# pierrepaleo/sift_pyocl

Hardware: AMD Instinct MI355X
Metric: SiftPlan.keypoints throughput, 4096x4096 fp32 (Mpix/s; keypoints/s in keypoints_per_s) (higher is better)
Workload: dtype f32

## Files before the change

### sift_pyocl_amd/csrc/k_extrema.hpp

```cpp
#pragma once
#include <hip/hip_runtime.h>
#include <stdint.h>
#include "siftmath.hpp"
#include "k_xcd.hpp"
#include <type_traits>

namespace siftk {

struct BlurPlanes { const float *p[6]; };

#define SIFT_EXT_ROWS 64
inline int extrema_strip_rows(int W, int H, int border, int min_strips = 2000) {
    const int nx = (W - 2 * border + 61) / 62;
    int rows = SIFT_EXT_ROWS;
    while (rows > 4 && (int64_t)nx * ((H - 2 * border + rows - 1) / rows) < min_strips) rows >>= 1;
    return rows;
}

__device__ __forceinline__ float dog_at(const BlurPlanes &b, int s, size_t pos) { return b.p[s][pos] - b.p[s + 1][pos]; }

#ifndef SIFT_EXT_WAVES
#define SIFT_EXT_WAVES 5
#endif
#define SIFT_EXT_BUF 128
template <int BUF> struct ExtWaveLdsT { float4 buf[BUF + 192]; };
using ExtWaveLds = ExtWaveLdsT<SIFT_EXT_BUF>;

struct RefineArgs {
    float peak_thresh, init_sigma;
    float4 *kp;
    int *kp_aux, *n_kp;
    int kp_capacity, oct;
    int *c_scale;
};
__device__ __forceinline__ void refine_candidates(const BlurPlanes &b, int W, int H, const float4 *__restrict__ cand, int n,
                                                  float peak_thresh, float init_sigma, float4 *__restrict__ kp,
                                                  int *__restrict__ kp_aux, int *__restrict__ n_kp, int kp_capacity, int oct,
                                                  int first, int stride, int *__restrict__ c_scale);

template <int BUF>
__device__ __forceinline__ void ext_store_pending(const ExtWaveLdsT<BUF> &L, float4 *__restrict__ cand, int capacity, int slot, int count, int lane) {
    __builtin_amdgcn_wave_barrier();
    for (int e = lane; e < count; e += 64)
        if (slot + e < capacity) cand[slot + e] = L.buf[e];
    __builtin_amdgcn_wave_barrier();
}

template <int BUF>
__device__ __forceinline__ void ext_edge_filter(const BlurPlanes &b, int W, float edth, ExtWaveLdsT<BUF> &L, int from, int &pending, int lane) {
    int out = from;
    __builtin_amdgcn_wave_barrier();
    for (int base = from; base < pending; base += 64) {
        const int e = base + lane;
        bool keep = false;
        float4 c = make_float4(0.f, 0.f, 0.f, 0.f);
        if (e < pending) {
            c = L.buf[e];
            const float val = c.x;
            const int s = (int)c.w;
            const size_t pc = (size_t)(int)c.y * W + (int)c.z;
            const float *pa = b.p[1], *pb = b.p[2];
            if (s == 2) { pa = b.p[2]; pb = b.p[3]; } else if (s == 3) { pa = b.p[3]; pb = b.p[4]; }
#define DOG_AT(o) (pa[pc + (o)] - pb[pc + (o)])
            const float up = DOG_AT(-(ptrdiff_t)W), dn = DOG_AT(W);
            const float lf = DOG_AT(-1), rt = DOG_AT(1);
            const float H00 = (float)(((double)up - 2.0 * (double)val) + (double)dn);
            const float H11 = (float)(((double)lf - 2.0 * (double)val) + (double)rt);
            const float dd = (DOG_AT(W + 1) - DOG_AT(W - 1)) - (DOG_AT(-(ptrdiff_t)W + 1) - DOG_AT(-(ptrdiff_t)W - 1));
#undef DOG_AT
            const float H01 = (float)((double)dd / 4.0);
            const float det = H00 * H11 - H01 * H01;
            const float tr = H00 + H11;
            keep = !(det < edth * tr * tr) && val != 0.0f;
        }
        __builtin_amdgcn_wave_barrier();
        const unsigned long long m = __ballot(keep);
        if (keep) L.buf[out + __popcll(m & ((1ull << lane) - 1ull))] = c;
        out += __popcll(m);
        __builtin_amdgcn_wave_barrier();
    }
    pending = out;
}

template <int BUF, bool REFINE = false>
__device__ __forceinline__ void extrema_strip(const BlurPlanes &b, int W, int H, int border, int rows, bool active, int sx, int sy,
                                              double contrast, float edth, float4 *__restrict__ cand, int *__restrict__ counter,
                                              int capacity, ExtWaveLdsT<BUF> &L, int &pending, const RefineArgs *ra = nullptr,
                                              int y_lo = -1, int y_hi = -1) {
    if (y_lo < 0) { y_lo = border; y_hi = H - border; }
    auto refine_parked = [&]() {
        __builtin_amdgcn_wave_barrier();
        refine_candidates(b, W, H, L.buf, pending, ra->peak_thresh, ra->init_sigma, ra->kp, ra->kp_aux, ra->n_kp, ra->kp_capacity,
                          ra->oct, threadIdx.x & 63, 64, ra->c_scale);
        __builtin_amdgcn_wave_barrier();
        pending = 0;
    };
    const int lane = threadIdx.x & 63;
    const int x = border + sx * 62 + lane - 1;
    const int xc = min(max(x, 0), W - 1);
    const bool col_ok = (lane >= 1) && (lane <= 62) && (x < W - border);
    const int ya = y_lo + sy * rows;
    const int yb = active ? min(ya + rows, y_hi) : ya - 2;
    int tested = pending;

    float cf = (float)contrast;
    if (!((double)cf > contrast)) cf = __uint_as_float(__float_as_uint(cf) + 1u);
    auto ld = [&](int k, unsigned off) { return *reinterpret_cast<const float *>(reinterpret_cast<const char *>(b.p[k]) + off); };
    auto from_left = [](float v) { return __int_as_float(__builtin_amdgcn_update_dpp(0, __float_as_int(v), 0x138, 0xf, 0xf, true)); };
    auto from_right = [](float v) { return __int_as_float(__builtin_amdgcn_update_dpp(0, __float_as_int(v), 0x130, 0xf, 0xf, true)); };

    float hM[3][3], hm[3][3];
    float ctr[3] = {0.f, 0.f, 0.f}, ctr_next[3];
#pragma unroll
    for (int r = 0; r < 3; r++)
#pragma unroll
        for (int k = 0; k < 3; k++) { hM[r][k] = 0.f; hm[r][k] = 0.f; }

    const unsigned pitch = (unsigned)W * 4u;
    unsigned off = ((unsigned)max(ya - 1, 0) * (unsigned)W + (unsigned)xc) * 4u;
    float vn[6];
    if (active) {
#pragma unroll
        for (int k = 0; k < 6; k++) vn[k] = ld(k, off);
    } else {
#pragma unroll
        for (int k = 0; k < 6; k++) vn[k] = 0.f;
    }
    for (int y = ya - 1; y <= yb; y++) {
        float v[6];
#pragma unroll
        for (int k = 0; k < 6; k++) v[k] = vn[k];
        if (y < yb) {
            off += pitch;
#pragma unroll
            for (int k = 0; k < 6; k++) vn[k] = ld(k, off);
        }
        float d[5];
#pragma unroll
        for (int k = 0; k < 5; k++) d[k] = v[k] - v[k + 1];
#pragma unroll
        for (int k = 0; k < 3; k++) { hM[0][k] = hM[1][k]; hM[1][k] = hM[2][k]; hm[0][k] = hm[1][k]; hm[1][k] = hm[2][k]; }
#pragma unroll
        for (int k = 0; k < 3; k++) {
            const float M = fmaxf(fmaxf(d[k], d[k + 1]), d[k + 2]);
            const float m = fminf(fminf(d[k], d[k + 1]), d[k + 2]);
            hM[2][k] = fmaxf(fmaxf(from_left(M), M), from_right(M));
            hm[2][k] = fminf(fminf(from_left(m), m), from_right(m));
            ctr_next[k] = d[k + 1];
        }
        bool found[3] = {false, false, false};
        const int yc = y - 1;
        if (y >= ya + 1 && col_ok) {
#pragma unroll
            for (int k = 0; k < 3; k++) {
                const float val = ctr[k];
                if (fabsf(val) >= cf) {
                    const float M27 = fmaxf(fmaxf(hM[0][k], hM[1][k]), hM[2][k]);
                    const float m27 = fminf(fminf(hm[0][k], hm[1][k]), hm[2][k]);
                    found[k] = (val > 0.0f) ? (val >= M27) : (val <= m27);
                }
            }
        }
#pragma unroll
        for (int k = 0; k < 3; k++) {
            const unsigned long long m = __ballot(found[k]);
            if (m) {
                if (found[k]) L.buf[pending + __popcll(m & ((1ull << lane) - 1ull))] = make_float4(ctr[k], (float)yc, (float)x, (float)(k + 1));
                pending += __popcll(m);
            }
        }
        if (pending > BUF) {
            ext_edge_filter(b, W, edth, L, tested, pending, lane);
            tested = 0;
            if (REFINE) refine_parked();
            else {
                int slot = 0;
                if (lane == 0) slot = atomicAdd(counter, pending);
                ext_store_pending(L, cand, capacity, __shfl(slot, 0), pending, lane);
                pending = 0;
            }
        }
#pragma unroll
        for (int k = 0; k < 3; k++) ctr[k] = ctr_next[k];
    }
    ext_edge_filter(b, W, edth, L, tested, pending, lane);
    if (REFINE) refine_parked();
}

template <bool REFINE>
__global__ __launch_bounds__(256) __attribute__((amdgpu_waves_per_eu(REFINE ? 4 : SIFT_EXT_WAVES, 8))) void extrema_kernel(BlurPlanes b, int W, int H, int border, int rows, double contrast,
                                                      float edth, float4 *__restrict__ cand,
                                                      int *__restrict__ counter, int capacity, RefineArgs ra,
                                                      int y_lo, int y_hi,
                                                      int xcd_map) {
    __shared__ ExtWaveLds lds_all[4];
    __shared__ int s_pending[4], s_base;
    const int lane = threadIdx.x & 63;
    ExtWaveLds &L = lds_all[threadIdx.x >> 6];
    if (y_lo < 0) { y_lo = border; y_hi = H - border; }
    const int nx = (W - 2 * border + 61) / 62;
    const int ny = (y_hi - y_lo + rows - 1) / rows;
    const int wg = xcd_map ? xcd_contiguous((int)blockIdx.x, (int)gridDim.x) : (int)blockIdx.x;
    const int wid = wg * 4 + (threadIdx.x >> 6);
    const bool active = wid < nx * ny;
    int pending = 0;
    extrema_strip<SIFT_EXT_BUF, REFINE>(b, W, H, border, rows, active, active ? wid % nx : 0, active ? wid / nx : 0, contrast, edth, cand,
                                        counter, capacity, L, pending, &ra, y_lo, y_hi);
    if (REFINE) return;
    if (lane == 0) s_pending[threadIdx.x >> 6] = pending;
    __syncthreads();
    if (threadIdx.x == 0) {
        const int tot = s_pending[0] + s_pending[1] + s_pending[2] + s_pending[3];
        s_base = tot ? atomicAdd(counter, tot) : 0;
    }
    __syncthreads();
    {
        const int w = threadIdx.x >> 6;
        int slot = s_base;
        for (int q = 0; q < w; q++) slot += s_pending[q];
        ext_store_pending(L, cand, capacity, slot, pending, lane);
    }
}

__device__ __forceinline__ void refine_candidates(const BlurPlanes &b, int W, int H, const float4 *__restrict__ cand, int n,
                                                  float peak_thresh, float init_sigma, float4 *__restrict__ kp,
                                                  int *__restrict__ kp_aux, int *__restrict__ n_kp, int kp_capacity, int oct,
                                                  int first, int stride, int *__restrict__ c_scale) {
    int seen[3] = {0, 0, 0};
    for (int i = first; i < n; i += stride) {
        const float4 k = cand[i];
        int r = (int)k.y, c = (int)k.z;
        const int scale = (int)k.w;
        if (r == -1) continue;
        seen[0] += scale <= 1; seen[1] += scale == 2; seen[2] += scale >= 3;
        const float *Pa = b.p[0], *Pb = b.p[1], *Pc = b.p[2], *Pd = b.p[3];
        if (scale == 2) { Pa = b.p[1]; Pb = b.p[2]; Pc = b.p[3]; Pd = b.p[4]; }
        else if (scale == 3) { Pa = b.p[2]; Pb = b.p[3]; Pc = b.p[4]; Pd = b.p[5]; }
        int newr = r, newc = c, moves = 5;
        bool again = true;
        float s0 = 0.f, s1 = 0.f, s2 = 0.f, peak = 0.f;
        while (again) {
            r = newr; c = newc;
            const size_t pos = (size_t)r * W + c;
#define DOGP(o) (Pa[pos + (o)] - Pb[pos + (o)])
#define DOGD(o) (Pb[pos + (o)] - Pc[pos + (o)])
#define DOGN(o) (Pc[pos + (o)] - Pd[pos + (o)])
            const float P0 = DOGP(0), D0 = DOGD(0), N0 = DOGN(0);
            const float Dd = DOGD(W), Du = DOGD(-W), Dr = DOGD(1), Dl = DOGD(-1);
            const float Pd_ = DOGP(W), Pu = DOGP(-W), Pr = DOGP(1), Pl = DOGP(-1);
            const float Nd = DOGN(W), Nu = DOGN(-W), Nr = DOGN(1), Nl = DOGN(-1);
            const float Ddr = DOGD(W + 1), Ddl = DOGD(W - 1), Dur = DOGD(-W + 1), Dul = DOGD(-W - 1);
#undef DOGP
#undef DOGD
#undef DOGN
            const float g0 = (N0 - P0) / 2.0f;
            const float g1 = (Dd - Du) / 2.0f;
            const float g2 = (Dr - Dl) / 2.0f;
            const float H00 = P0 - 2.0f * D0 + N0;
            const float H11 = Du - 2.0f * D0 + Dd;
            const float H22 = Dl - 2.0f * D0 + Dr;
            const float H01 = ((Nd - Nu) - (Pd_ - Pu)) / 4.0f;
            const float H02 = ((Nr - Nl) - (Pr - Pl)) / 4.0f;
            const float H12 = ((Ddr - Ddl) - (Dur - Dul)) / 4.0f;
            const float H10 = H01, H20 = H02, H21 = H12;
            const float det = -(H02 * H11 * H20) + H01 * H12 * H20 + H02 * H10 * H21
                              - H00 * H12 * H21 - H01 * H10 * H22 + H00 * H11 * H22;
            const float K00 = H11 * H22 - H12 * H21;
            const float K01 = H02 * H21 - H01 * H22;
            const float K02 = H01 * H12 - H02 * H11;
            const float K10 = H12 * H20 - H10 * H22;
            const float K11 = H00 * H22 - H02 * H20;
            const float K12 = H02 * H10 - H00 * H12;
            const float K20 = H10 * H21 - H11 * H20;
            const float K21 = H01 * H20 - H00 * H21;
            const float K22 = H00 * H11 - H01 * H10;
            s0 = -(g0 * K00 + g1 * K01 + g2 * K02) / det;
            s1 = -(g0 * K10 + g1 * K11 + g2 * K12) / det;
            s2 = -(g0 * K20 + g1 * K21 + g2 * K22) / det;
            peak = D0 + 0.5f * (s0 * g0 + s1 * g1 + s2 * g2);
            if (s1 > 0.6f && newr < H - 3) newr++;
            else if (s1 < -0.6f && newr > 3) newr--;
            if (s2 > 0.6f && newc < W - 3) newc++;
            else if (s2 < -0.6f && newc > 3) newc--;
            if (moves > 0 && (newr != r || newc != c)) moves--;
            else again = false;
        }
        if (fabsf(s0) <= 1.5f && fabsf(s1) <= 1.5f && fabsf(s2) <= 1.5f && fabsf(peak) >= peak_thresh) {
            const float sig = init_sigma * siftmath::exp2f_(((float)scale + s0) / 3.0f);
            const int slot = atomicAdd(n_kp, 1);
            if (slot < kp_capacity) {
                kp[slot] = make_float4(peak, (float)r + s1, (float)c + s2, sig);
                kp_aux[slot] = scale | (oct << 8);
            }
        }
    }
    if (c_scale) {
#pragma unroll
        for (int q = 0; q < 3; q++) {
            int t = seen[q];
#pragma unroll
            for (int off = 32; off > 0; off >>= 1) t += __shfl_xor(t, off);
            if (t && (threadIdx.x & 63) == q) atomicAdd(c_scale + q, t);
        }
    }
}

__global__ __launch_bounds__(256) void refine_kernel(BlurPlanes b, int W, int H, const float4 *__restrict__ cand,
                                                     const int *__restrict__ n_cand, int cand_capacity,
                                                     float peak_thresh, float init_sigma,
                                                     float4 *__restrict__ kp, int *__restrict__ kp_aux,
                                                     int *__restrict__ n_kp, int kp_capacity, int oct,
                                                     int *__restrict__ c_scale) {
    const int n = min(*n_cand, cand_capacity);
    refine_candidates(b, W, H, cand, n, peak_thresh, init_sigma, kp, kp_aux, n_kp, kp_capacity, oct,
                      blockIdx.x * blockDim.x + threadIdx.x, gridDim.x * blockDim.x, c_scale);
}

__global__ void compact_kernel(const float4 *__restrict__ in, float4 *__restrict__ out, int *__restrict__ counter,
                               int start, int end, int capacity) {
    for (int i = start + blockIdx.x * blockDim.x + threadIdx.x; i < end; i += gridDim.x * blockDim.x) {
        const float4 k = in[i];
        if (k.y != -1.0f) {
            const int slot = atomicAdd(counter, 1);
            if (slot < capacity) out[slot] = k;
        }
    }
}

__global__ void dog_kernel(const float *__restrict__ a, const float *__restrict__ bnext, float *__restrict__ out, int64_t n) {
    const int64_t stride = (int64_t)gridDim.x * blockDim.x;
    for (int64_t i = (int64_t)blockIdx.x * blockDim.x + threadIdx.x; i < n; i += stride)
        out[i] = -1.0f * bnext[i] + 1.0f * a[i];
}

}
```

Measured before the change: 22190.

## Hand-schedule extrema row scan with DPP max/min, SGPR masks and 3-way unroll

Result: no change. 22170 (median of 2 runs) (-0.1%).

```diff
diff --git a/sift_pyocl_amd/csrc/k_extrema.hpp b/sift_pyocl_amd/csrc/k_extrema.hpp
--- a/sift_pyocl_amd/csrc/k_extrema.hpp
+++ b/sift_pyocl_amd/csrc/k_extrema.hpp
@@ -99,22 +99,51 @@
     const int x = border + sx * 62 + lane - 1;
     const int xc = min(max(x, 0), W - 1);
     const bool col_ok = (lane >= 1) && (lane <= 62) && (x < W - border);
-    const int ya = y_lo + sy * rows;
-    const int yb = active ? min(ya + rows, y_hi) : ya - 2;
+    const int ya = __builtin_amdgcn_readfirstlane(y_lo + sy * rows);
+    const int yb = __builtin_amdgcn_readfirstlane(active ? min(ya + rows, y_hi) : ya - 2);
+    pending = __builtin_amdgcn_readfirstlane(pending);
     int tested = pending;
 
     float cf = (float)contrast;
     if (!((double)cf > contrast)) cf = __uint_as_float(__float_as_uint(cf) + 1u);
     auto ld = [&](int k, unsigned off) { return *reinterpret_cast<const float *>(reinterpret_cast<const char *>(b.p[k]) + off); };
-    auto from_left = [](float v) { return __int_as_float(__builtin_amdgcn_update_dpp(0, __float_as_int(v), 0x138, 0xf, 0xf, true)); };
-    auto from_right = [](float v) { return __int_as_float(__builtin_amdgcn_update_dpp(0, __float_as_int(v), 0x130, 0xf, 0xf, true)); };
-
-    float hM[3][3], hm[3][3];
-    float ctr[3] = {0.f, 0.f, 0.f}, ctr_next[3];
+    auto window_row = [](const float (&d)[5], float (&M)[3], float (&m)[3]) {
+        float t0, t1, t2, t3, t4, t5;
+        asm("v_max3_f32 %6, %12, %13, %14\n\t"
+            "v_min3_f32 %7, %12, %13, %14\n\t"
+            "v_max3_f32 %8, %13, %14, %15\n\t"
+            "v_min3_f32 %9, %13, %14, %15\n\t"
+            "v_max3_f32 %10, %14, %15, %16\n\t"
+            "v_min3_f32 %11, %14, %15, %16\n\t"
+            "v_max_f32_dpp %0, %6, %6 wave_shr:1 row_mask:0xf bank_mask:0xf bound_ctrl:1\n\t"
+            "v_min_f32_dpp %1, %7, %7 wave_shr:1 row_mask:0xf bank_mask:0xf bound_ctrl:1\n\t"
+            "v_max_f32_dpp %2, %8, %8 wave_shr:1 row_mask:0xf bank_mask:0xf bound_ctrl:1\n\t"
+            "v_min_f32_dpp %3, %9, %9 wave_shr:1 row_mask:0xf bank_mask:0xf bound_ctrl:1\n\t"
+            "v_max_f32_dpp %4, %10, %10 wave_shr:1 row_mask:0xf bank_mask:0xf bound_ctrl:1\n\t"
+            "v_min_f32_dpp %5, %11, %11 wave_shr:1 row_mask:0xf bank_mask:0xf bound_ctrl:1\n\t"
+            "v_max_f32_dpp %0, %6, %0 wave_shl:1 row_mask:0xf bank_mask:0xf bound_ctrl:1\n\t"
+            "v_min_f32_dpp %1, %7, %1 wave_shl:1 row_mask:0xf bank_mask:0xf bound_ctrl:1\n\t"
+            "v_max_f32_dpp %2, %8, %2 wave_shl:1 row_mask:0xf bank_mask:0xf bound_ctrl:1\n\t"
+            "v_min_f32_dpp %3, %9, %3 wave_shl:1 row_mask:0xf bank_mask:0xf bound_ctrl:1\n\t"
+            "v_max_f32_dpp %4, %10, %4 wave_shl:1 row_mask:0xf bank_mask:0xf bound_ctrl:1\n\t"
+            "v_min_f32_dpp %5, %11, %5 wave_shl:1 row_mask:0xf bank_mask:0xf bound_ctrl:1"
+            : "=&v"(M[0]), "=&v"(m[0]), "=&v"(M[1]), "=&v"(m[1]), "=&v"(M[2]), "=&v"(m[2]),
+              "=&v"(t0), "=&v"(t1), "=&v"(t2), "=&v"(t3), "=&v"(t4), "=&v"(t5)
+            : "v"(d[0]), "v"(d[1]), "v"(d[2]), "v"(d[3]), "v"(d[4]));
+    };
+    auto max3 = [](float a, float b2, float c2) { float r; asm("v_max3_f32 %0, %1, %2, %3" : "=v"(r) : "v"(a), "v"(b2), "v"(c2)); return r; };
+    auto min3 = [](float a, float b2, float c2) { float r; asm("v_min3_f32 %0, %1, %2, %3" : "=v"(r) : "v"(a), "v"(b2), "v"(c2)); return r; };
+    auto mask_ge = [](float a, float b2) { unsigned long long r; asm("v_cmp_ge_f32_e64 %0, %1, %2" : "=s"(r) : "v"(a), "v"(b2)); return r; };
+    auto mask_le = [](float a, float b2) { unsigned long long r; asm("v_cmp_le_f32_e64 %0, %1, %2" : "=s"(r) : "v"(a), "v"(b2)); return r; };
+    auto mask_abs_ge = [](float a, float b2) { unsigned long long r; asm("v_cmp_ge_f32_e64 %0, |%1|, %2" : "=s"(r) : "v"(a), "v"(b2)); return r; };
+    auto mask_pos = [](float a) { unsigned long long r; asm("v_cmp_lt_f32_e64 %0, 0, %1" : "=s"(r) : "v"(a)); return r; };
+    const unsigned long long cols = __ballot(col_ok);
+
+    float hM[3][3], hm[3][3], c[3][3];
 #pragma unroll
     for (int r = 0; r < 3; r++)
 #pragma unroll
-        for (int k = 0; k < 3; k++) { hM[r][k] = 0.f; hm[r][k] = 0.f; }
+        for (int k = 0; k < 3; k++) { hM[r][k] = 0.f; hm[r][k] = 0.f; c[r][k] = 0.f; }
 
     const unsigned pitch = (unsigned)W * 4u;
     unsigned off = ((unsigned)max(ya - 1, 0) * (unsigned)W + (unsigned)xc) * 4u;
@@ -126,46 +155,34 @@
 #pragma unroll
         for (int k = 0; k < 6; k++) vn[k] = 0.f;
     }
-    for (int y = ya - 1; y <= yb; y++) {
-        float v[6];
-#pragma unroll
-        for (int k = 0; k < 6; k++) v[k] = vn[k];
+    auto row = [&](auto slot, int y) {
+        constexpr int S = decltype(slot)::value, CS = (S + 2) % 3;
+        float d[5];
+#pragma unroll
+        for (int k = 0; k < 5; k++) d[k] = vn[k] - vn[k + 1];
+        asm volatile("" : "+v"(d[0]), "+v"(d[1]), "+v"(d[2]), "+v"(d[3]), "+v"(d[4]));
         if (y < yb) {
             off += pitch;
 #pragma unroll
             for (int k = 0; k < 6; k++) vn[k] = ld(k, off);
         }
-        float d[5];
-#pragma unroll
-        for (int k = 0; k < 5; k++) d[k] = v[k] - v[k + 1];
-#pragma unroll
-        for (int k = 0; k < 3; k++) { hM[0][k] = hM[1][k]; hM[1][k] = hM[2][k]; hm[0][k] = hm[1][k]; hm[1][k] = hm[2][k]; }
+        window_row(d, hM[S], hm[S]);
+#pragma unroll
+        for (int k = 0; k < 3; k++) c[S][k] = d[k + 1];
+        const int yc = y - 1;
+        const unsigned long long here = (y >= ya + 1) ? cols : 0ull;
 #pragma unroll
         for (int k = 0; k < 3; k++) {
-            const float M = fmaxf(fmaxf(d[k], d[k + 1]), d[k + 2]);
-            const float m = fminf(fminf(d[k], d[k + 1]), d[k + 2]);
-            hM[2][k] = fmaxf(fmaxf(from_left(M), M), from_right(M));
-            hm[2][k] = fminf(fminf(from_left(m), m), from_right(m));
-            ctr_next[k] = d[k + 1];
-        }
-        bool found[3] = {false, false, false};
-        const int yc = y - 1;
-        if (y >= ya + 1 && col_ok) {
-#pragma unroll
-            for (int k = 0; k < 3; k++) {
-                const float val = ctr[k];
-                if (fabsf(val) >= cf) {
-                    const float M27 = fmaxf(fmaxf(hM[0][k], hM[1][k]), hM[2][k]);
-                    const float m27 = fminf(fminf(hm[0][k], hm[1][k]), hm[2][k]);
-                    found[k] = (val > 0.0f) ? (val >= M27) : (val <= m27);
+            const float val = c[CS][k];
+            const float M27 = max3(hM[0][k], hM[1][k], hM[2][k]);
+            const float m27 = min3(hm[0][k], hm[1][k], hm[2][k]);
+            const unsigned long long pos = mask_pos(val);
+            const unsigned long long m = here & mask_abs_ge(val, cf) & ((pos & mask_ge(val, M27)) | (~pos & mask_le(val, m27)));
+            if (m) {
+                if (__builtin_amdgcn_inverse_ballot_w64(m)) {
+                    const int before = __builtin_amdgcn_mbcnt_hi((unsigned)(m >> 32), __builtin_amdgcn_mbcnt_lo((unsigned)m, 0u));
+                    L.buf[pending + before] = make_float4(val, (float)yc, (float)x, (float)(k + 1));
                 }
-            }
-        }
-#pragma unroll
-        for (int k = 0; k < 3; k++) {
-            const unsigned long long m = __ballot(found[k]);
-            if (m) {
-                if (found[k]) L.buf[pending + __popcll(m & ((1ull << lane) - 1ull))] = make_float4(ctr[k], (float)yc, (float)x, (float)(k + 1));
                 pending += __popcll(m);
             }
         }
@@ -174,14 +191,21 @@
             tested = 0;
             if (REFINE) refine_parked();
             else {
-                int slot = 0;
-                if (lane == 0) slot = atomicAdd(counter, pending);
-                ext_store_pending(L, cand, capacity, __shfl(slot, 0), pending, lane);
+                int slot0 = 0;
+                if (lane == 0) slot0 = atomicAdd(counter, pending);
+                ext_store_pending(L, cand, capacity, __shfl(slot0, 0), pending, lane);
                 pending = 0;
             }
-        }
-#pragma unroll
-        for (int k = 0; k < 3; k++) ctr[k] = ctr_next[k];
+            pending = __builtin_amdgcn_readfirstlane(pending);
+        }
+    };
+    for (int y = ya - 1; y <= yb;) {
+        row(std::integral_constant<int, 0>{}, y);
+        if (++y > yb) break;
+        row(std::integral_constant<int, 1>{}, y);
+        if (++y > yb) break;
+        row(std::integral_constant<int, 2>{}, y);
+        ++y;
     }
     ext_edge_filter(b, W, edth, L, tested, pending, lane);
     if (REFINE) refine_parked();
```
